# drtconway/zotmer

Measured on AMD Instinct MI355X. Metric: Gk-mers/sec kmerize k=25 on synthetic 150bp FASTQ; achieved HBM GB/s fraction, higher is better.
Workload: dtype u64

## Files before the change

include/zotk.h:

```cpp
#ifndef ZOTK_H
#define ZOTK_H

#include <stdint.h>

#ifdef __cplusplus
extern "C" {
#endif

#define ZK_OK 0
#define ZK_EINVAL (-1)
#define ZK_ENOMEM (-2)
#define ZK_EHIP (-3)
#define ZK_ENOSPC (-4)
#define ZK_EOVERFLOW (-5)
#define ZK_EINTERNAL (-6)
#define ZK_ERANGE (-7)

typedef struct zk_ctx zk_ctx;

zk_ctx* zk_create(int device, uint64_t workspace_bytes);
void zk_destroy(zk_ctx* ctx);
const char* zk_last_error(zk_ctx* ctx);
int zk_set_stream(zk_ctx* ctx, void* hip_stream);
void* zk_get_stream(zk_ctx* ctx);
// ... 9 lines not shown
int zk_host_alloc(zk_ctx* ctx, uint64_t bytes, void** ptr);
int zk_host_free(zk_ctx* ctx, void* ptr);
int zk_upload_async(zk_ctx* ctx, void* d_dst, const void* src, uint64_t bytes);

#define ZK_TUNE_SORT_VARIANT 1
#define ZK_TUNE_PAIRS_VARIANT 2
#define ZK_TUNE_SHORT_SORT 3
#define ZK_TUNE_XCD_GROUP 5
#define ZK_TUNE_SIDE_DIV 4
#define ZK_TUNE_EARLY_COLLAPSE 7
#define ZK_TUNE_PACKED_PAIRS 8
#define ZK_TUNE_WIDE_TILES 9
#define ZK_TUNE_STREAM_PASS 10
#define ZK_TUNE_STREAM_RANGES 11
#define ZK_TUNE_TAG_WORDS 12
#define ZK_TUNE_DEDUPE_VARIANT 13
#define ZK_TUNE_DEDUPE_LIMIT 14
#define ZK_TUNE_DEDUPE_BITS 15
#define ZK_TUNE_COMM_CHUNK 6
#define ZK_TUNE_TAG_PASS 17
#define ZK_TUNE_KWAY 18
#define ZK_TUNE_TILE_SORT 19
#define ZK_TUNE_STRAND_BLOCKS 20
#define ZK_TUNE_COMM_SELF_LOOP 16
int zk_tune(zk_ctx* ctx, int what, int value);

#define ZK_PROF_HIST_STREAM 1
#define ZK_PROF_HIST_ARRAY 2
#define ZK_PROF_PASS_STREAM 3
#define ZK_PROF_PASS_KEYS 4
#define ZK_PROF_PASS_PAIRS 5
#define ZK_PROF_RLE 6
#define ZK_PROF_UNION 7
#define ZK_PROF_SELECT 8
#define ZK_PROF_MIRROR 9
#define ZK_PROF_INTERSECT 10
#define ZK_PROF_COUNT_HIST 11
#define ZK_PROF_PASS_PACKED 12
#define ZK_PROF_SAMPLE 13
#define ZK_PROF_TILE_SORT 14
#define ZK_PROF_CAPTURE_HITS 15
#define ZK_PROF_PROJECT_SUM 16
#define ZK_PROF_SPECTRUM 17
#define ZK_PROF_STRAND_KEYS 18
#define ZK_PROF_STRAND_PAIRS 19
#define ZK_PROF_FORMAT_PAIRS 20
// ... 259 lines not shown
```

zotmer_amd/csrc/context.hip:

```cpp
#include <stdarg.h>
#include <string.h>

#include "internal.hpp"
#include <vector>

namespace zk {

int fail(zk_ctx* c, int code, const char* fmt, ...) {
    char buf[512];
    va_list ap;
    va_start(ap, fmt);
    vsnprintf(buf, sizeof buf, fmt, ap);
    va_end(ap);
    if (c) c->last_error = buf;
    return code;
}

void arena_reset(zk_ctx* c) { c->arena_off = 0; }

int arena_alloc(zk_ctx* c, uint64_t bytes, void** p) {
    const uint64_t need = (bytes + 255) & ~255ull;
    if (c->arena_off + need > c->arena_size) {
        if (c->arena_off != 0)
            return fail(c, ZK_ENOMEM, "workspace too small: %llu bytes in use, %llu more needed, %llu reserved (call zk_reserve)",
// ... 285 lines not shown
    if (what == ZK_TUNE_SHORT_SORT) { c->short_sort = value; return ZK_OK; }
    if (what == ZK_TUNE_SIDE_DIV) { c->side_div = value; return ZK_OK; }
    if (what == ZK_TUNE_WIDE_TILES) { c->wide_tiles = value ? 1 : 0; return ZK_OK; }
    if (what == ZK_TUNE_PACKED_PAIRS) { c->packed_pairs = value ? 1 : 0; return ZK_OK; }
    if (what == ZK_TUNE_EARLY_COLLAPSE) { c->early_collapse = value < 0 ? 0 : (value > 3 ? 3 : value); return ZK_OK; }
    if (what == ZK_TUNE_COMM_SELF_LOOP) { c->comm_self_loop = value ? 1 : 0; return ZK_OK; }
    if (what == ZK_TUNE_COMM_CHUNK) { c->comm_chunk_bytes = value > 0 ? (uint64_t)value : 0; return ZK_OK; }
    if (what == ZK_TUNE_STREAM_PASS) {
#ifdef ZK_PHASES
        c->stream_pass = value < 0 ? 0 : value;
#else
        if (value < 0 || value > 3) return fail(c, ZK_EINVAL, "stream pass variant %d (0, 1, 2 or 3)", value);
        c->stream_pass = value;
#endif
        return ZK_OK;
    }
    if (what == ZK_TUNE_TAG_WORDS) { c->tag_words = value < 0 ? 0 : (value > 2 ? 2 : value); return ZK_OK; }
    if (what == ZK_TUNE_DEDUPE_VARIANT) { c->dedupe_variant = value < 0 ? -1 : (value & 3); return ZK_OK; }
    if (what == ZK_TUNE_KWAY) { c->kway = value < 0 ? 0 : (value > 2 ? 2 : value); return ZK_OK; }
    if (what == ZK_TUNE_TILE_SORT) { c->tile_sort = value ? 1 : 0; return ZK_OK; }
    if (what == ZK_TUNE_TAG_PASS) { c->tag_pass = value ? 1 : 0; return ZK_OK; }
    if (what == ZK_TUNE_DEDUPE_BITS) { c->dedupe_bits = value < 0 ? 0 : value; return ZK_OK; }
    if (what == ZK_TUNE_STRAND_BLOCKS) { c->strand_blocks = value < 0 ? 0 : (value > 3 ? 1 : value); return ZK_OK; }
    if (what == ZK_TUNE_DEDUPE_LIMIT) { c->dedupe_limit = value < 1 ? 1 : (value > 65536 ? 65536 : value); return ZK_OK; }
    if (what == ZK_TUNE_STREAM_RANGES) { c->stream_ranges = value < 0 ? 0 : (value > 4096 ? 4096 : value); return ZK_OK; }
    if (what == ZK_TUNE_XCD_GROUP) {
        if (value < 0 || value > 32 || (value & (value - 1))) return fail(c, ZK_EINVAL, "xcd group must be 0 or a power of two <= 32");
        c->xcd_group = value;
        return ZK_OK;
    }
    return fail(c, ZK_EINVAL, "unknown tuning knob %d", what);
}

int zk_debug_buffer(zk_ctx* c, void* d_buf) {
    if (!c) return ZK_EINVAL;
    enter(c);
    c->dbg = (u64*)d_buf;
    return ZK_OK;
}

int zk_profile(zk_ctx* c, int enable) {
    if (!c) return ZK_EINVAL;
    enter(c);
    ZK_HIP(c, hipStreamSynchronize(c->stream));
    for (auto& r : c->prof) { (void)hipEventDestroy(r.a); (void)hipEventDestroy(r.b); }
    c->prof.clear();
// ... 91 lines not shown
```

zotmer_amd/csrc/dedupe2.hip:

```cpp
#include "dedupe.hpp"
#include <type_traits>

namespace zk {

template <int BLOCK_, int BATCH_, int ITEMS_>
struct Dedupe2Smem {
    static constexpr int BLOCK = BLOCK_, BATCH = BATCH_, ITEMS = ITEMS_, TILE = BLOCK * ITEMS, NW = BLOCK / 64, ALL = 11264, SPT = ALL / BLOCK,
                         NB = 1024, SIDE = 64 + 64 * BATCH;
    static_assert(ALL % BLOCK == 0 && ALL % 8 == 0 && ITEMS % BATCH == 0 && ITEMS % 4 == 0, "whole rounds, whole quads, whole batches");
    alignas(16) u32 keys[ALL];
    alignas(16) u32 cnt[ALL / 2];
    union {
        u32 side[NW][SIDE];
        struct { u32 bc[NB]; u32 bbase[NB + 1]; } g;
    };
    u32 ticket;
    u32 nout;
};

template <int ITEMS>
struct Dedupe2Next {
    u32 chunk;
    u64 lo;
    u32 len;
// ... 283 lines not shown
        st.len = nhi - nlo < (u64)a.limit ? (u32)(nhi - nlo) : ~0u;
    }
    if (st.len - 1u < ~0u - 1u) dedupe2_load<BLOCK, ITEMS, TAGIN>(a, st.lo, 0, st.len, tmask, st.tag);
    __syncthreads();
    u32 ph[8] = {0, 0, 0, 0, 0, 0, 0, 0};
    u32 tlast = a.dbg ? (u32)__builtin_amdgcn_s_memtime() : 0u;
    (void)tlast;
    u32 nblk = 0;
    while (st.chunk < a.chunks) {
        dedupe2_block<BLOCK, BATCH, ITEMS, TAGIN, UNSORTED>(a, sm, st, ph, tlast);
        __syncthreads();
        DD_PHASE(6);
        nblk++;
    }
    if (a.dbg && threadIdx.x == 0 && blockIdx.x < 256) {
        for (int k = 0; k < 8; k++) a.dbg[(u64)blockIdx.x * 16 + k] = ph[k];
        a.dbg[(u64)blockIdx.x * 16 + 8] = nblk;
    }
}

int launch_dedupe2(zk_ctx* c, const DedupeArgs& a, bool tagin, int variant, bool unsorted) {
    const u32 want = 2u * (u32)c->num_cus;
    const u32 grid = a.chunks < want ? a.chunks : want;
#define ZK_DD2(N, T, U) hipLaunchKernelGGL((dedupe2_kernel<512, N, 8, T, U>), dim3(grid), dim3(512), 0, c->stream, a)
#define ZK_DD2B(T, U) switch (variant & 3) { case 1: ZK_DD2(1, T, U); break; case 2: ZK_DD2(2, T, U); break; default: ZK_DD2(4, T, U); break; }
    if (unsorted) {
        if (tagin) ZK_DD2B(true, true) else ZK_DD2B(false, true)
    } else {
        if (tagin) ZK_DD2B(true, false) else ZK_DD2B(false, false)
    }
#undef ZK_DD2B
#undef ZK_DD2
    ZK_HIP(c, hipGetLastError());
    return ZK_OK;
}

}
```

zotmer_amd/csrc/internal.hpp:

```cpp
#pragma once
#include <hip/hip_runtime.h>
#include <stddef.h>
#include <stdint.h>
#include <stdio.h>
#include <string>
#include <vector>

#include "../../include/zotk.h"
#include "common.hpp"

struct zk_strand_counters { u32 n_declined, fail; };
struct zk_scalars {
    u64 rle_side;
    u64 total;
    u64 acgt[4];
    u64 n_keys;
    u64 rec_info[3];
    u64 sample_n;
    u64 dedupe_flags, dedupe_n_retry, dedupe_counter, dedupe_n_big, dedupe_n_bad;
    u64 dedupe_n_in;
    u64 dedupe_n_out;
    zk_strand_counters strand;
    u64 hist_big_n;
    u64 capture_kept;
// ... 44 lines not shown
              ZK_SPAN(dedupe_flags, dedupe_n_bad) == 5 * sizeof(u64), "dedupe_pass clears and reads its five words as one range");

struct zk_ctx {
    int device = 0;
    hipStream_t stream = nullptr;
    bool own_stream = false;
    int num_cus = 256;
    int sort_variant = 3;
    int short_sort = 0;
    int packed_pairs = 1;
    int wide_tiles = 1;
    int early_collapse = 1;
    int side_div = 8;
    int pairs_variant = 7;
    int stream_pass = 1;
    int tag_words = 2;
    int dedupe_variant = 0;
    int dedupe_limit = 65536;
    int tag_pass = 0;
    int kway = 1;
    int tile_sort = 1;
    int dedupe_bits = 0;
    int strand_blocks = 1;
    int stream_ranges = 0;

    char* arena = nullptr;
    uint64_t arena_size = 0;
    uint64_t arena_off = 0;

    char* aux = nullptr;
    uint64_t aux_size = 0;

    u64* status = nullptr;
    uint64_t status_words = 0;
    unsigned short* part16 = nullptr;
    uint64_t part16_words = 0;
    u32 epoch = 0;
    u32* d_ticket = nullptr;
    u32* d_xticket = nullptr;
    int num_xcd = 1;
    int xcd_group = 0;
    u32 ticket_base = 0;

    u32* d_err = nullptr;
    zk_scalars* d_scalars = nullptr;
    zk_scalars* h_scalars = nullptr;
// ... 73 lines not shown
        p.shift[i] = s;
        s += p.bits[i];
    }
    return p;
}
int sort_keys(zk_ctx* c, u64* keys, u64* alt, uint64_t n, int key_bits, u64** result);
int sort_pairs(zk_ctx* c, u64* keys, u64* alt, u32* vals, u32* valt, uint64_t n, int key_bits, u64** rk, u32** rv);
int sort_keys_upper(zk_ctx* c, u64* keys, u64* alt, uint64_t n, int key_bits, int lo_bit, u64** result, int prof_tag = ZK_PROF_PASS_PACKED);
int sort_pairs_upper(zk_ctx* c, u64* keys, u64* alt, u32* vals, u32* valt, uint64_t n, int key_bits, int lo_bit, u64** rk, u32** rv);
int sort_pairs_mirrored(zk_ctx* c, const u64* src_k, const u32* src_v, u64* keys, u64* alt, u32* vals, u32* valt, uint64_t n, int K,
                        u64** rk, u32** rv, int lo_bit = 0);
int sort_pairs_rbits(zk_ctx* c);
struct StreamSample { int shift; uint64_t value; double max_ratio; uint64_t seen = 0, distinct = 0; bool want_distinct = false; };
struct StreamTags { bool written = false; u64* cuts = nullptr; uint32_t blocks = 0; };
struct StreamSrc { const u8* stream; uint64_t n_bytes; int K; int mode; int lo_bit; int hi_bit = 0; StreamSample* sample = nullptr;
                   StreamTags* tags = nullptr; };
int sort_stream(zk_ctx* c, const StreamSrc& src, u64* buf_a, u64* buf_b, uint64_t cap, uint64_t* n_keys,
                uint64_t acgt[4], u64** result);
int sort_rbits(zk_ctx* c);
PassPlan sort_plan_upper(zk_ctx* c, int key_bits, int lo_bit);
int sort_first_bits(zk_ctx* c, int key_bits, int lo_bit);
constexpr int MIRROR_RBITS = 9, MIRROR_RADIX = 1 << MIRROR_RBITS;
struct MirrorHist { int passes; int shift[4]; int bits[4]; u64* raw; };
int sort_keys_upper_counted(zk_ctx* c, u64* keys, u64* alt, uint64_t n, int key_bits, int lo_bit, u64* counted, u64** result);
struct DedupeResult {
    uint64_t n_out = 0;
    uint32_t flags = 0;
    uint32_t n_big = 0;
    u64 *cuts = nullptr, *nwords = nullptr, *incl = nullptr, *big = nullptr, *work = nullptr;
    u32* sub = nullptr;
    uint32_t chunks = 0;
    int pack = 0;
    int tag_bits = 0;
    bool unsorted = false;
};
int dedupe_pass(zk_ctx* c, const u64* keys, uint64_t n, int key_bits, int b, int pack, u64* work, uint64_t cap, DedupeResult* r,
                uint64_t* n_in = nullptr, uint64_t max_chunks = 0, const u32* tags = nullptr, const u64* tag_cuts = nullptr,
                bool unsorted = false);
int expand_tags(zk_ctx* c, const u32* tags, const u64* cuts, uint32_t blocks, int tag_bits, u64* keys_out, uint64_t first_block = 0, uint64_t n_blocks = 0);
int dedupe_finish(zk_ctx* c, const DedupeResult& r, u64* out_k, u32* out_c, u64* out_m = nullptr, int K = 0, int gbases = 0,
                  u64** mirror_hist = nullptr, int* mirror_group_bits = nullptr, bool packed_out = false);
int dedupe_sort_blocks(zk_ctx* c, DedupeResult& r);
int strand_blocks(zk_ctx* c, const DedupeResult& r, u64* keys_buf, uint64_t buf_words, int K, u64* out_k, u32* out_c, uint64_t cap,
                  uint64_t* n_out);
int collapse_pass(zk_ctx* c, const u64* keys, uint64_t n, int shift, int bits, int pack, u64* out, uint64_t cap, uint64_t* n_out,
                  uint64_t max_tiles = 0);
struct StreamRows { u32* rows = nullptr; u64* offs = nullptr; u32 ranges = 0, radix = 0; u32* gcodes = nullptr; u16* gvalid = nullptr;
// ... 61 lines not shown
```

zotmer_amd/csrc/radix_sort.hip:

```cpp
#include <stdlib.h>
#include "internal.hpp"
#include "encode_tile.hpp"

namespace zk {

constexpr int MAX_RADIX = 1024;

enum { SRC_ARRAY = 0, SRC_STREAM = 1 };

template <int BLOCK_, int ITEMS_, int RBITS_, int ROUNDS_ = 1, int WPE_ = 1, int SEG_ = 32, bool PIPE_ = false>
struct Cfg {
    static constexpr int BLOCK = BLOCK_, ITEMS = ITEMS_, RBITS = RBITS_, ROUNDS = ROUNDS_, WPE = WPE_, SEG = SEG_;
    static constexpr bool PIPE = PIPE_;
    static_assert(SEG == 0 || (BLOCK * ITEMS < 32768 && (SEG & (SEG - 1)) == 0), "16-bit tile counts");
    static constexpr int TILE = BLOCK * ITEMS, RADIX = 1 << RBITS, NW = BLOCK / 64;
    static constexpr int EXCH = TILE / ROUNDS, IPR = ITEMS / ROUNDS;
    static_assert(ITEMS % ROUNDS == 0, "ROUNDS");
    static constexpr int DPT = (RADIX + BLOCK - 1) / BLOCK;
    static_assert(ITEMS % 2 == 0 && 2 * ITEMS < 256, "ITEMS");
    static_assert(64 * ITEMS < 65536, "per-wave ranks are 16-bit");
    static_assert(RADIX <= MAX_RADIX && RBITS * MAX_PASSES >= 64, "RBITS");
};

struct SortArgs {
// ... 1207 lines not shown
        if (SRC == SRC_STREAM && src.n_bytes) {
            h.rec_info = c->d_scalars->rec_info;
            ZK_HIP(c, hipMemsetAsync(h.rec_info, 0, 3 * sizeof(u64), c->stream));
            hipLaunchKernelGGL(first_newline_kernel, dim3(1), dim3(256), 0, c->stream, src.stream, (u64)src.n_bytes, h.rec_info);
        }
        if (acgt) ZK_HIP(c, hipMemsetAsync(acgt, 0, sizeof(u64) * 4, c->stream));
        u32 grid = grid_cap(c, h.tiles, 8);
        if (grid == 0) grid = 1;
        prof_begin(c, SRC == SRC_STREAM ? ZK_PROF_HIST_STREAM : ZK_PROF_HIST_ARRAY, SRC == SRC_STREAM ? src.n_bytes : 8 * src.n);
        if constexpr (SRC == SRC_STREAM && C::ITEMS == 16 && C::BLOCK <= 512) {
            if (src.mode != ZK_KEYS_BOTH) hipLaunchKernelGGL((hist_kernel<C, SRC, true>), dim3(grid), dim3(C::BLOCK), 0, c->stream, h);
            else hipLaunchKernelGGL((hist_kernel<C, SRC, false>), dim3(grid), dim3(C::BLOCK), 0, c->stream, h);
        } else {
            hipLaunchKernelGGL((hist_kernel<C, SRC, false>), dim3(grid), dim3(C::BLOCK), 0, c->stream, h);
        }
        prof_end(c);
        ZK_HIP(c, hipGetLastError());
        hipLaunchKernelGGL(hist_scan_kernel, dim3(1), dim3(256), 0, c->stream, ghist, plan.passes, (int)C::RADIX, d_n);
        ZK_HIP(c, hipGetLastError());
        return ZK_OK;
    }

    static int sort_keys(zk_ctx* c, u64* keys, u64* alt, uint64_t n, int key_bits, u64** result, int lo_bit = 0, int prof_tag = 0,
                         u64* counted = nullptr) {
        PassPlan plan = make_plan(key_bits - lo_bit, C::RBITS, lo_bit);
        u64* ghist = counted;
        if (!counted) ZK_TRY(arena_alloc(c, sizeof(u64) * MAX_PASSES * C::RADIX, (void**)&ghist));
        SortArgs a = {};
        a.kin = keys; a.n = n;
        a.prof_tag = prof_tag;
        if (counted) {
            hipLaunchKernelGGL(hist_scan_kernel, dim3(1), dim3(256), 0, c->stream, ghist, plan.passes, (int)C::RADIX, &c->d_scalars->n_keys);
            ZK_HIP(c, hipGetLastError());
        } else {
            ZK_TRY(launch_hist<SRC_ARRAY>(c, a, plan, ghist, nullptr, &c->d_scalars->n_keys));
        }
        u64* in = keys; u64* out = alt;
        for (int p = 0; p < plan.passes; p++) {
            a.kin = in; a.kout = out; a.shift = plan.shift[p]; a.bits = plan.bits[p];
            a.ghist = ghist + p * C::RADIX;
            ZK_TRY(launch_keys_pass(c, a));
            u64* t = in; in = out; out = t;
        }
        *result = in;
        return ZK_OK;
    }

    static int sort_pairs(zk_ctx* c, u64* keys, u64* alt, u32* vals, u32* valt, uint64_t n, int key_bits, u64** rk, u32** rv,
                          const u64* src_k = nullptr, const u32* src_v = nullptr, int mirror_K = 0, int lo_bit = 0, bool unordered = false) {
        PassPlan plan = make_plan(key_bits - lo_bit, C::RBITS, lo_bit);
        u64* ghist;
        ZK_TRY(arena_alloc(c, sizeof(u64) * MAX_PASSES * C::RADIX, (void**)&ghist));
        SortArgs a = {};
        a.kin = mirror_K ? src_k : keys; a.n = n; a.mirror_K = mirror_K;
        ZK_TRY(launch_hist<SRC_ARRAY>(c, a, plan, ghist, nullptr, &c->d_scalars->n_keys));
        const u64* in = mirror_K ? src_k : keys; const u32* vi = mirror_K ? src_v : vals;
        u64* out = mirror_K ? keys : alt; u32* vo = mirror_K ? vals : valt;
        for (int p = 0; p < plan.passes; p++) {
            a.kin = in; a.kout = out; a.vin = vi; a.vout = vo; a.shift = plan.shift[p]; a.bits = plan.bits[p];
            a.ghist = ghist + p * C::RADIX;
            a.mirror_K = (p == 0) ? mirror_K : 0;
            if constexpr (PIPE_PAIRS) {
                a.straddle = nullptr;
// ... 208 lines not shown

int sort_pairs(zk_ctx* c, u64* keys, u64* alt, u32* vals, u32* valt, uint64_t n, int key_bits, u64** rk, u32** rv) {
    *rk = keys; *rv = vals;
    if (n == 0) return ZK_OK;
    const int top = c->tile_sort ? tile_sort_top_bits(n, key_bits, sort_pairs_rbits(c)) : 0;
    if (top) {
        u64* k1 = nullptr; u32* v1 = nullptr;
        bool declined = false;
        ZK_TRY(sort_pairs_upper(c, keys, alt, vals, valt, n, key_bits, key_bits - top, &k1, &v1));
        ZK_TRY(tile_sort(c, k1, v1, n, key_bits, top, &declined));
        *rk = k1; *rv = v1;
        if (!declined) return ZK_OK;
        return sort_pairs_lsd(c, k1, k1 == keys ? alt : keys, v1, v1 == vals ? valt : vals, n, key_bits, rk, rv);
    }
    return sort_pairs_lsd(c, keys, alt, vals, valt, n, key_bits, rk, rv);
}

int sort_keys_upper(zk_ctx* c, u64* keys, u64* alt, uint64_t n, int key_bits, int lo_bit, u64** result, int prof_tag) {
    *result = keys;
    if (n == 0 || lo_bit >= key_bits) return ZK_OK;
    ZK_SORT_DISPATCH(c, sort_keys(c, keys, alt, n, key_bits, result, lo_bit, prof_tag));
}

int sort_keys_upper_counted(zk_ctx* c, u64* keys, u64* alt, uint64_t n, int key_bits, int lo_bit, u64* counted, u64** result) {
    *result = keys;
    if (n == 0 || lo_bit >= key_bits) return ZK_OK;
    return Sorter<V3>::sort_keys(c, keys, alt, n, key_bits, result, lo_bit, ZK_PROF_PASS_PACKED, counted);
}

int sort_pairs_upper(zk_ctx* c, u64* keys, u64* alt, u32* vals, u32* valt, uint64_t n, int key_bits, int lo_bit, u64** rk, u32** rv) {
    *rk = keys; *rv = vals;
    if (n == 0) return ZK_OK;
    ZK_PAIRS_DISPATCH(c, sort_pairs(c, keys, alt, vals, valt, n, key_bits, rk, rv, nullptr, nullptr, 0, lo_bit));
}

int sort_pairs_mirrored(zk_ctx* c, const u64* src_k, const u32* src_v, u64* keys, u64* alt, u32* vals, u32* valt, uint64_t n, int K,
                        u64** rk, u32** rv, int lo_bit) {
    *rk = keys; *rv = vals;
    if (n == 0) return ZK_OK;
    ZK_PAIRS_DISPATCH(c, sort_pairs(c, keys, alt, vals, valt, n, 2 * K, rk, rv, src_k, src_v, K, lo_bit, true));
}

int sort_rbits(zk_ctx* c) { ZK_SORT_DISPATCH(c, rbits()); }
int sort_pairs_rbits(zk_ctx* c) { ZK_PAIRS_DISPATCH(c, rbits()); }

PassPlan sort_plan_upper(zk_ctx* c, int key_bits, int lo_bit) { return make_plan(key_bits - lo_bit, sort_rbits(c), lo_bit); }

int sort_first_bits(zk_ctx* c, int key_bits, int lo_bit) {
    if (lo_bit >= key_bits) return 0;
    return make_plan(key_bits - lo_bit, sort_rbits(c), lo_bit).bits[0];
// ... 14 lines not shown
```

zotmer_amd/csrc/strand_blocks.hip:

```cpp
#include "tile_group.hpp"

namespace zk {

constexpr int SB_ITEMS = 16, SB_GROUPS = 2048;
constexpr u32 SB_GROUP_MAX = 128;
typedef TileSortSmem<SB_ITEMS, SB_GROUPS, false> StrandSmem;
constexpr int SB_BLOCK_BITS = 18;

__global__ __launch_bounds__(256) void strand_mirror_kernel(const u64* __restrict__ in, const u64* __restrict__ cuts, const u64* __restrict__ incl,
                                                            const u64* __restrict__ nwords, u32 chunks, int pack, int K, u64* __restrict__ out_m,
                                                            MirrorHist mh) {
    __shared__ u32 bins[4 * 512];
    const bool hist = mh.passes > 0;
    if (hist) {
        for (int q = threadIdx.x; q < 4 * 512; q += blockDim.x) bins[q] = 0;
        __syncthreads();
    }
    const u64 maxc = (1ull << pack) - 1;
    for (u32 v = blockIdx.x; v < chunks; v += gridDim.x) {
        const u64 cnt = nwords[v];
        const u64 dst0 = incl[v] - cnt;
        const u64* src = in + cuts[v];
        for (u64 i0 = threadIdx.x; i0 < cnt; i0 += 4ull * blockDim.x) {
            u64 w4[4];
#pragma unroll
            for (int q = 0; q < 4; q++) {
                const u64 i = i0 + (u64)q * blockDim.x;
                w4[q] = i < cnt ? src[i] : 0;
            }
// ... 22 lines not shown
    const u32 g = blockIdx.x * blockDim.x + threadIdx.x;
    if (g > (1u << SB_BLOCK_BITS)) return;
    u64 lo = 0, hi = n;
    if (g == (1u << SB_BLOCK_BITS)) lo = n;
    while (lo < hi) {
        const u64 mid = (lo + hi) >> 1;
        if ((m[mid] >> shift) < (u64)g) lo = mid + 1; else hi = mid;
    }
    start[g] = lo;
}

struct StrandArgs {
    const u64* cw;
    const u64* cuts; const u64* nwords; const u64* incl;
    const u64* m;
    const u64* mstart;
    u64* ok; u32* oc;
    int pack;
    int pshift;
    u32* n_declined;
    u32* declined;
};

__device__ __forceinline__ bool strand_crowded(const StrandSmem& sm, int tid) {
    static_assert(SB_GROUPS == 4 * TS_BLOCK, "four groups a thread");
    u32 big = 0;
#pragma unroll
    for (int q = 0; q < 4; q++) big |= sm.start[4 * tid + q + 1] - sm.start[4 * tid + q] > SB_GROUP_MAX ? 1u : 0u;
    return __syncthreads_or((int)big) != 0;
}

__device__ __forceinline__ void strand_write(const StrandSmem& sm, const TileMap& tm, u32 m, u64* ok, u32* oc, int pack, int tid) {
    const u64 maxc = (1ull << pack) - 1;
    constexpr int E = 2;
    for (u32 i0 = (u32)tid; i0 < m; i0 += E * TS_BLOCK) {
        u32 i[E], place[E];
        u64 mine[E];
#pragma unroll
        for (int e = 0; e < E; e++) i[e] = i0 + e * TS_BLOCK;
        tile_rank<E, false>(sm, tm, i, m, mine, place);
#pragma unroll
        for (int e = 0; e < E; e++) {
            if (i[e] >= m) break;
            ok[place[e]] = mine[e] >> pack;
            oc[place[e]] = (u32)(mine[e] & maxc);
        }
    }
}

__global__ __launch_bounds__(TS_BLOCK, 2 * TS_BLOCK / 256) void strand_block_union_kernel(StrandArgs a) {
    using S = StrandSmem;
    constexpr u32 CAP = S::CAP;
    static_assert(sizeof(S) <= 80 * 1024, "two workgroups per CU");
    __shared__ S sm;
    const u32 b = blockIdx.x;
    const u64 nc = a.nwords[b], m0 = a.mstart[b], nm = a.mstart[b + 1] - m0;
    const u64 n = nc + nm;
    if (n == 0) return;
    if (n > CAP) {
        if (threadIdx.x == 0) a.declined[atomicAdd(a.n_declined, 1u)] = b;
        return;
    }
    int tid = threadIdx.x;
    asm volatile("" : "+v"(tid));
    const u32 m = (u32)n;
    const TileMap tm = tile_group<SB_ITEMS, SB_GROUPS, false>(sm, a.cw, nullptr, a.cuts[b], m, a.pshift, tid, a.m, m0, (u32)nc);
    if (strand_crowded(sm, tid)) {
        if (tid == 0) a.declined[atomicAdd(a.n_declined, 1u)] = b;
        return;
    }
    const u64 out0 = a.incl[b] - nc + m0;
    strand_write(sm, tm, m, a.ok + out0, a.oc + out0, a.pack, tid);
}

constexpr int SB_SPLIT = 256;
struct StrandBigSmem {
    StrandSmem t;
    u64 sp[SB_SPLIT];
    u32 cnt[SB_SPLIT + 2];
    u32 tile[SB_SPLIT + 2];
    u32 ntiles, gcount, fail;
};

__global__ __launch_bounds__(TS_BLOCK) void strand_big_block_kernel(StrandArgs a, u32 n_list, u64* __restrict__ scratch, u32* __restrict__ fail) {
    using S = StrandBigSmem;
    constexpr u32 CAP = StrandSmem::CAP, R = SB_SPLIT + 1;
    __shared__ S sm;
    u64* gat = scratch + (u64)blockIdx.x * CAP;
    const int lane = threadIdx.x & 63;
    for (u32 li = blockIdx.x; li < n_list; li += gridDim.x) {
        int tid = threadIdx.x;
        asm volatile("" : "+v"(tid));
        const u32 b = a.declined[li];
        const u64 nc = a.nwords[b], m0 = a.mstart[b], nm = a.mstart[b + 1] - m0, n = nc + nm;
        const u64* C = a.cw + a.cuts[b];
// ... 122 lines not shown
    if (uc == 0) return ZK_OK;
    if (!(K & 1) || r.n_big || r.chunks != (1u << SB_BLOCK_BITS)) return fail(c, ZK_EINTERNAL, "strand_blocks: K %d, %u big counts, %u blocks", K, r.n_big, r.chunks);
    const uint64_t a8w = ((8 * uc + 255) & ~255ull) / 8;
    if (2 * a8w > buf_words) return fail(c, ZK_EINTERNAL, "strand_blocks: %llu words do not fit twice in %llu", (unsigned long long)uc, (unsigned long long)buf_words);
    if (2 * uc > cap) return fail(c, ZK_ENOSPC, "output holds %llu entries, the table has %llu", (unsigned long long)cap, (unsigned long long)(2 * uc));
    const int pk = r.pack, key_bits = 2 * K + pk, lo_bit = key_bits - SB_BLOCK_BITS;
    u64* mw = keys_buf;
    u64* malt = keys_buf + a8w;
    MirrorHist mh = {};
    if (c->sort_variant == 3) {
        const PassPlan plan = sort_plan_upper(c, key_bits, lo_bit);
        if (plan.passes <= 4) {
            ZK_TRY(arena_alloc(c, sizeof(u64) * MAX_PASSES * 512, (void**)&mh.raw));
            ZK_HIP(c, hipMemsetAsync(mh.raw, 0, sizeof(u64) * MAX_PASSES * 512, c->stream));
            mh.passes = plan.passes;
            for (int p = 0; p < plan.passes; p++) { mh.shift[p] = plan.shift[p]; mh.bits[p] = plan.bits[p]; }
        }
    }
    prof_begin(c, ZK_PROF_SELECT, 16 * uc);
    hipLaunchKernelGGL(strand_mirror_kernel, dim3((u32)c->num_cus * 8), dim3(256), 0, c->stream, r.work, r.cuts, r.incl, r.nwords, r.chunks, pk, K, mw, mh);
    prof_end(c);
    ZK_HIP(c, hipGetLastError());
    u64* sk = nullptr;
    if (mh.passes) ZK_TRY(sort_keys_upper_counted(c, mw, malt, uc, key_bits, lo_bit, mh.raw, &sk));
    else ZK_TRY(sort_keys_upper(c, mw, malt, uc, key_bits, lo_bit, &sk));
    u64* mstart;
    u32* declined;
    ZK_TRY(arena_alloc(c, sizeof(u64) * ((1ull << SB_BLOCK_BITS) + 1), (void**)&mstart));
    ZK_TRY(arena_alloc(c, sizeof(u32) * r.chunks, (void**)&declined));
    StrandArgs a = {};
    a.cw = r.work; a.cuts = r.cuts; a.nwords = r.nwords; a.incl = r.incl; a.m = sk; a.mstart = mstart;
    a.ok = out_k; a.oc = out_c; a.pack = pk; a.pshift = lo_bit;
    a.n_declined = &c->d_scalars->strand.n_declined;
    a.declined = declined;
    u32* fail = &c->d_scalars->strand.fail;
    prof_begin(c, ZK_PROF_UNION, 8 * 2 * uc + 12 * 2 * uc);
    hipLaunchKernelGGL(strand_starts_kernel, dim3(((1u << SB_BLOCK_BITS) + 256) / 256), dim3(256), 0, c->stream, sk, (u64)uc, lo_bit, mstart);
    ZK_HIP(c, hipMemsetAsync(&c->d_scalars->strand, 0, sizeof(zk_strand_counters), c->stream));
    hipLaunchKernelGGL(strand_block_union_kernel, dim3(r.chunks), dim3(TS_BLOCK), 0, c->stream, a);
    prof_end(c);
    ZK_HIP(c, hipGetLastError());
    ZK_TRY(fetch(c, &c->h_scalars->strand));
    ZK_TRY(check_device_error(c));
    const uint32_t n_declined = c->h_scalars->strand.n_declined;
    bool other_way = n_declined && c->strand_blocks == 3;
    if (n_declined && !other_way) {
        const uint32_t grid = n_declined < 2u * (uint32_t)c->num_cus ? n_declined : 2u * (uint32_t)c->num_cus;
        u64* scratch;
        ZK_TRY(arena_alloc(c, sizeof(u64) * StrandSmem::CAP * grid, (void**)&scratch));
        prof_begin(c, ZK_PROF_UNION, 0);
        hipLaunchKernelGGL(strand_big_block_kernel, dim3(grid), dim3(TS_BLOCK), 0, c->stream, a, n_declined, scratch, fail);
        prof_end(c);
        ZK_HIP(c, hipGetLastError());
        ZK_TRY(fetch(c, &c->h_scalars->strand));
        ZK_TRY(check_device_error(c));
        other_way = c->h_scalars->strand.fail != 0;
    }
    if (!other_way) {
        *n_out = 2 * uc;
        return ZK_OK;
    }
    DedupeResult rs = r;
// ... 11 lines not shown
```

zotmer_amd/csrc/tile_group.hpp:

```cpp
#pragma once
#include "internal.hpp"

namespace zk {

constexpr int TS_BLOCK = 512;
constexpr u32 TS_SLACK = 1024;

template <int ITEMS, int GROUPS, bool PAIRS>
struct TileSortSmem {
    static constexpr int CAP = TS_BLOCK * ITEMS;
    alignas(16) u64 keys[CAP];
    u32 vals[PAIRS ? CAP : 1];
    u16 idx[PAIRS ? CAP : 1];
    alignas(16) u32 start[GROUPS + 8];
    u32 wsum[TS_BLOCK / 64];
};
struct TileMap {
    u64 kmin; int sh; u32 scale;
    __device__ __forceinline__ u32 group(u64 key) const {
        const u32 d = (u32)((key - kmin) >> sh);
        return scale ? __umulhi(d, scale) : d;
    }
};

template <int ITEMS, int G, bool PAIRS, class S>
__device__ __forceinline__ TileMap tile_group(S& sm, const u64* kin, const u32* vin, u64 lo, u32 m, int pshift, int tid,
                                              const u64* kin2 = nullptr, u64 lo2 = 0, u32 m1 = ~0u, bool ranged = false, u64 vlo = 0,
                                              u64 vhi = 0) {
    constexpr int NW = TS_BLOCK / 64, QPT = G / TS_BLOCK / 4;
    static_assert(QPT == 1 || QPT == 2, "four or eight groups a thread in the scan");
    static_assert((S::CAP <= 8192 || (!PAIRS && S::CAP <= 16384)) && G <= 4096, "group | place << 12 in a word; u16 places of pairs");
    const int lane = tid & 63, wave = __builtin_amdgcn_readfirstlane(tid >> 6);
    const u64* kp = kin + lo;
    u64 k[ITEMS];
    u32 v[PAIRS ? ITEMS : 1];
#pragma unroll
    for (int j = 0; j < ITEMS; j++) {
        const u32 i = (u32)j * TS_BLOCK + tid;
        k[j] = i < m ? (i < m1 ? kp[i] : kin2[lo2 + (i - m1)]) : ~0ull;
        if constexpr (PAIRS) v[j] = i < m ? vin[lo + i] : 0u;
    }
    u64 first, last;
    if (ranged) { first = vlo; last = vhi; pshift = 0; }
    else { first = m1 ? kp[0] : kin2[lo2]; last = m - 1 < m1 ? kp[m - 1] : kin2[lo2 + (m - 1 - m1)]; }
    TileMap tm;
    tm.kmin = (first >> pshift) << pshift;
    const u64 rm1 = (((last >> pshift) - (first >> pshift)) << pshift) | ((1ull << pshift) - 1ull);
    tm.sh = rm1 >> 32 ? 32 - __builtin_clzll(rm1) : 0;
    const u32 rs = (u32)(rm1 >> tm.sh);
    tm.scale = rs < (u32)G ? 0u : (u32)(((u64)G << 32) / ((u64)rs + 1ull));
    {
        uint4* z = reinterpret_cast<uint4*>(sm.start);
#pragma unroll
        for (int q = 0; q < QPT; q++) z[QPT * tid + q] = make_uint4(0, 0, 0, 0);
    }
    __syncthreads();
    u32 gp[ITEMS];
#pragma unroll
    for (int j = 0; j < ITEMS; j++) {
        const u32 i = (u32)j * TS_BLOCK + tid;
        const u32 g = i < m ? tm.group(k[j]) : 0u;
        gp[j] = g;
        if (i < m) gp[j] |= atomicAdd(&sm.start[g], 1u) << 12;
    }
    __syncthreads();
    {
        uint4* z = reinterpret_cast<uint4*>(sm.start);
        uint4 cq[QPT];
        u32 sum = 0;
#pragma unroll
        for (int q = 0; q < QPT; q++) { cq[q] = z[QPT * tid + q]; sum += cq[q].x + cq[q].y + cq[q].z + cq[q].w; }
        const u32 inc = wave_incl_scan_u32(sum);
        if (lane == 63) sm.wsum[wave] = inc;
        __syncthreads();
        u32 run = inc - sum;
#pragma unroll
        for (int w = 0; w < NW; w++) run += w < wave ? sm.wsum[w] : 0u;
#pragma unroll
        for (int q = 0; q < QPT; q++) {
            uint4 sq;
            sq.x = run; run += cq[q].x; sq.y = run; run += cq[q].y; sq.z = run; run += cq[q].z; sq.w = run; run += cq[q].w;
            z[QPT * tid + q] = sq;
        }
        if (tid == 0) sm.start[G] = m;
    }
    __syncthreads();
#pragma unroll
    for (int j = 0; j < ITEMS; j++) {
        const u32 i = (u32)j * TS_BLOCK + tid;
        if (i < m) {
            const u32 p = sm.start[gp[j] & (G - 1)] + (gp[j] >> 12);
            sm.keys[p] = k[j];
            if constexpr (PAIRS) { sm.vals[p] = v[j]; sm.idx[p] = (u16)i; }
        }
    }
    __syncthreads();
    return tm;
}

template <int E, bool PAIRS, class S>
__device__ __forceinline__ void tile_rank(const S& sm, const TileMap& tm, const u32 (&i)[E], u32 m, u64 (&mine)[E], u32 (&place)[E]) {
    constexpr u32 CAP = S::CAP;
    auto before = [&](u64 ko, u32 q, u64 km, u32 at) -> bool {
        if (ko != km) return ko < km;
        if constexpr (PAIRS) return q != at && sm.idx[q] < sm.idx[at];
        else return q < at;
    };
    u32 g0[E], g1[E];
#pragma unroll
    for (int e = 0; e < E; e++) mine[e] = sm.keys[i[e] < m ? i[e] : 0u];
#pragma unroll
    for (int e = 0; e < E; e++) {
// ... 33 lines not shown
```

zotmer_amd/native.py:

```python
import ctypes as C
import os

import numpy as np

_HERE = os.path.dirname(os.path.abspath(__file__))
LIB_PATH = os.environ.get("ZOTK_LIB") or os.path.join(_HERE, "libzotk.so")

ZK_OK, ZK_EINVAL, ZK_ENOMEM, ZK_EHIP, ZK_ENOSPC, ZK_EOVERFLOW, ZK_EINTERNAL, ZK_ERANGE = 0, -1, -2, -3, -4, -5, -6, -7
KMERIZE_CANONICAL, KMERIZE_BOTH, KMERIZE_SUBSAMPLE, KMERIZE_CANONICAL_ONLY = 0, 1, 2, 4
STRAND_ORPHANS = 1
PROBE_TILE, PROBE_MAX_WINDOWS = 4096, 1024
TALLY_TILE = 2048
CONTIG_TILE = 4096
VARS_TILE = 4096
LINKS_TILE = 1024
NO_LINK = 0xFFFFFFFF
PILEUP_DIAGS, PILEUP_TILE = 256, 4096
PATH_TILE, PATH_CHUNK = 4096, 256
DEFAULT_TAG_WORDS = 2

_ERRNAMES = {-1: "ZK_EINVAL", -2: "ZK_ENOMEM", -3: "ZK_EHIP", -4: "ZK_ENOSPC", -5: "ZK_EOVERFLOW",
             -6: "ZK_EINTERNAL", -7: "ZK_ERANGE"}


class ZotkError(RuntimeError):
    def __init__(self, code, msg):
        super().__init__("%s: %s" % (_ERRNAMES.get(code, code), msg))
        self.code = code


class Spectrum(C.Structure):
    _fields_ = [("n_shared", C.c_uint64), ("s_min", C.c_uint64), ("x_shared", C.c_uint64), ("y_shared", C.c_uint64),
                ("s_xy_lo", C.c_uint64), ("s_xy_hi", C.c_uint64), ("s_sqrt", C.c_double), ("s_js", C.c_double)]


class StrandStats(C.Structure):
    _fields_ = [("n_pairs", C.c_uint64), ("n_orphans", C.c_uint64), ("n_palindromes", C.c_uint64)]


class ContigStats(C.Structure):
    _fields_ = [("n_records", C.c_uint64), ("n_windows", C.c_uint64), ("n_keys", C.c_uint64), ("n_bins", C.c_uint64)]

# ... 351 lines not shown
        return cut.value

    def device_to_file(self, arr, fileno, offset, threads=None):
        self._check(self.lib.zk_device_to_file(self.h, arr.ptr, arr.nbytes, int(fileno), int(offset), threads or self.IO_THREADS))

    def file_to_device(self, fileno, offset, nbytes, dtype=np.uint8, threads=None):
        dt = np.dtype(dtype)
        out = self.empty(nbytes // dt.itemsize, dt)
        self._check(self.lib.zk_file_to_device(self.h, int(fileno), int(offset), int(nbytes), out.ptr, threads or self.IO_THREADS))
        return out

    def upload_stream(self, data):
        a = np.frombuffer(data, dtype=np.uint8) if isinstance(data, (bytes, bytearray, memoryview)) else np.asarray(data, np.uint8)
        return self.upload(a)

    PROF_TAGS = {"hist_stream": 1, "hist_array": 2, "pass_stream": 3, "pass_keys": 4, "pass_pairs": 5, "rle": 6,
                 "union_sum": 7, "select": 8, "mirror": 9, "intersect": 10, "count_hist": 11, "pass_packed": 12, "sample": 13, "tile_sort": 14,
                 "capture_hits": 15, "project_sum": 16, "spectrum": 17, "strand_keys": 18, "strand_pairs": 19, "format_pairs": 20,
                 "probe_scan": 21, "bait_tally": 22, "vars_scan": 23, "links": 24, "links_rc": 25, "contig_render": 26,
                 "pileup": 27, "pileup_cut": 28, "pulldown_tally": 29, "capture_kmers": 30, "path_scan": 31}

    TUNE_IDS = dict(sort_variant=1, pairs_variant=2, short_sort=3, side_div=4, xcd_group=5, comm_chunk=6, early_collapse=7,
                    packed_pairs=8, wide_tiles=9, stream_pass=10, stream_ranges=11, tag_words=12, dedupe_variant=13, dedupe_limit=14,
                    dedupe_bits=15, comm_self_loop=16, tag_pass=17, kway=18, tile_sort=19, strand_blocks=20)

    def tune(self, **knobs):
        for name in knobs:
            if name not in self.TUNE_IDS:
                raise TypeError("tune() got an unexpected keyword argument %r" % name)
        for name, value in knobs.items():
            if value is not None:
                self._check(self.lib.zk_tune(self.h, self.TUNE_IDS[name], int(value)))

    def profile(self, enable=True):
        self._check(self.lib.zk_profile(self.h, int(enable)))

    def profile_read(self):
        out = {}
        for name, tag in self.PROF_TAGS.items():
            n, b, ms = C.c_uint64(0), C.c_uint64(0), C.c_double(0)
            self._check(self.lib.zk_profile_read(self.h, tag, C.byref(n), C.byref(ms), C.byref(b)))
            if n.value:
                out[name] = dict(launches=n.value, ms=ms.value, bytes=b.value)
        return out

    def pack_reads(self, bases, offs):
        n_reads = offs.n - 1
# ... 575 lines not shown
```

Measured before the change: 165.2.

## Add strand_wide knob: unordered upper sort straddle, 1024-thread strand and dedupe kernels

Adds a strand_wide tuning knob with three bits. Bit 1, on by default, makes the strand path's upper-bits key sort run unordered and build straddle bitmaps for its first two passes. Bits 2 and 4, off by default, switch the unsorted dedupe and strand block-union kernels to 1024-thread workgroups, and tile_group is generalised over block size to support them. The default path aims to drop ordering work in the strand sort, at the cost of extra bitmap allocation and launches.

```diff
diff --git a/include/zotk.h b/include/zotk.h
--- a/include/zotk.h
+++ b/include/zotk.h
@@ -55,6 +55,7 @@
 #define ZK_TUNE_KWAY 18
 #define ZK_TUNE_TILE_SORT 19
 #define ZK_TUNE_STRAND_BLOCKS 20
+#define ZK_TUNE_STRAND_WIDE 21
 #define ZK_TUNE_COMM_SELF_LOOP 16
 int zk_tune(zk_ctx* ctx, int what, int value);
 
diff --git a/zotmer_amd/csrc/context.hip b/zotmer_amd/csrc/context.hip
--- a/zotmer_amd/csrc/context.hip
+++ b/zotmer_amd/csrc/context.hip
@@ -331,6 +331,7 @@
     if (what == ZK_TUNE_TAG_PASS) { c->tag_pass = value ? 1 : 0; return ZK_OK; }
     if (what == ZK_TUNE_DEDUPE_BITS) { c->dedupe_bits = value < 0 ? 0 : value; return ZK_OK; }
     if (what == ZK_TUNE_STRAND_BLOCKS) { c->strand_blocks = value < 0 ? 0 : (value > 3 ? 1 : value); return ZK_OK; }
+    if (what == ZK_TUNE_STRAND_WIDE) { c->strand_wide = value < 0 ? 0 : (value & 7); return ZK_OK; }
     if (what == ZK_TUNE_DEDUPE_LIMIT) { c->dedupe_limit = value < 1 ? 1 : (value > 65536 ? 65536 : value); return ZK_OK; }
     if (what == ZK_TUNE_STREAM_RANGES) { c->stream_ranges = value < 0 ? 0 : (value > 4096 ? 4096 : value); return ZK_OK; }
     if (what == ZK_TUNE_XCD_GROUP) {
diff --git a/zotmer_amd/csrc/dedupe2.hip b/zotmer_amd/csrc/dedupe2.hip
--- a/zotmer_amd/csrc/dedupe2.hip
+++ b/zotmer_amd/csrc/dedupe2.hip
@@ -329,6 +329,12 @@
 int launch_dedupe2(zk_ctx* c, const DedupeArgs& a, bool tagin, int variant, bool unsorted) {
     const u32 want = 2u * (u32)c->num_cus;
     const u32 grid = a.chunks < want ? a.chunks : want;
+    if (unsorted && (c->strand_wide & 2)) {
+        if (tagin) hipLaunchKernelGGL((dedupe2_kernel<1024, 2, 8, true, true>), dim3(grid), dim3(1024), 0, c->stream, a);
+        else hipLaunchKernelGGL((dedupe2_kernel<1024, 2, 8, false, true>), dim3(grid), dim3(1024), 0, c->stream, a);
+        ZK_HIP(c, hipGetLastError());
+        return ZK_OK;
+    }
 #define ZK_DD2(N, T, U) hipLaunchKernelGGL((dedupe2_kernel<512, N, 8, T, U>), dim3(grid), dim3(512), 0, c->stream, a)
 #define ZK_DD2B(T, U) switch (variant & 3) { case 1: ZK_DD2(1, T, U); break; case 2: ZK_DD2(2, T, U); break; default: ZK_DD2(4, T, U); break; }
     if (unsorted) {
diff --git a/zotmer_amd/csrc/internal.hpp b/zotmer_amd/csrc/internal.hpp
--- a/zotmer_amd/csrc/internal.hpp
+++ b/zotmer_amd/csrc/internal.hpp
@@ -90,6 +90,7 @@
     int tile_sort = 1;
     int dedupe_bits = 0;
     int strand_blocks = 1;
+    int strand_wide = 1;
     int stream_ranges = 0;
 
     char* arena = nullptr;
@@ -209,7 +210,8 @@
 int sort_first_bits(zk_ctx* c, int key_bits, int lo_bit);
 constexpr int MIRROR_RBITS = 9, MIRROR_RADIX = 1 << MIRROR_RBITS;
 struct MirrorHist { int passes; int shift[4]; int bits[4]; u64* raw; };
-int sort_keys_upper_counted(zk_ctx* c, u64* keys, u64* alt, uint64_t n, int key_bits, int lo_bit, u64* counted, u64** result);
+int sort_keys_upper_counted(zk_ctx* c, u64* keys, u64* alt, uint64_t n, int key_bits, int lo_bit, u64* counted, u64** result,
+                            bool unordered = false);
 struct DedupeResult {
     uint64_t n_out = 0;
     uint32_t flags = 0;
diff --git a/zotmer_amd/csrc/radix_sort.hip b/zotmer_amd/csrc/radix_sort.hip
--- a/zotmer_amd/csrc/radix_sort.hip
+++ b/zotmer_amd/csrc/radix_sort.hip
@@ -1253,7 +1253,7 @@
     }
 
     static int sort_keys(zk_ctx* c, u64* keys, u64* alt, uint64_t n, int key_bits, u64** result, int lo_bit = 0, int prof_tag = 0,
-                         u64* counted = nullptr) {
+                         u64* counted = nullptr, bool unordered = false) {
         PassPlan plan = make_plan(key_bits - lo_bit, C::RBITS, lo_bit);
         u64* ghist = counted;
         if (!counted) ZK_TRY(arena_alloc(c, sizeof(u64) * MAX_PASSES * C::RADIX, (void**)&ghist));
@@ -1270,6 +1270,9 @@
         for (int p = 0; p < plan.passes; p++) {
             a.kin = in; a.kout = out; a.shift = plan.shift[p]; a.bits = plan.bits[p];
             a.ghist = ghist + p * C::RADIX;
+            a.straddle = nullptr;
+            if (C::PIPE && unordered && p <= 1)
+                ZK_TRY(straddle_bitmap(c, n, keys_pass_tile(c), p == 1 ? ghist : nullptr, 1u << plan.bits[0], (u32)C::RADIX, &a.straddle));
             ZK_TRY(launch_keys_pass(c, a));
             u64* t = in; in = out; out = t;
         }
@@ -1524,10 +1527,10 @@
     ZK_SORT_DISPATCH(c, sort_keys(c, keys, alt, n, key_bits, result, lo_bit, prof_tag));
 }
 
-int sort_keys_upper_counted(zk_ctx* c, u64* keys, u64* alt, uint64_t n, int key_bits, int lo_bit, u64* counted, u64** result) {
+int sort_keys_upper_counted(zk_ctx* c, u64* keys, u64* alt, uint64_t n, int key_bits, int lo_bit, u64* counted, u64** result, bool unordered) {
     *result = keys;
     if (n == 0 || lo_bit >= key_bits) return ZK_OK;
-    return Sorter<V3>::sort_keys(c, keys, alt, n, key_bits, result, lo_bit, ZK_PROF_PASS_PACKED, counted);
+    return Sorter<V3>::sort_keys(c, keys, alt, n, key_bits, result, lo_bit, ZK_PROF_PASS_PACKED, counted, unordered);
 }
 
 int sort_pairs_upper(zk_ctx* c, u64* keys, u64* alt, u32* vals, u32* valt, uint64_t n, int key_bits, int lo_bit, u64** rk, u32** rv) {
diff --git a/zotmer_amd/csrc/strand_blocks.hip b/zotmer_amd/csrc/strand_blocks.hip
--- a/zotmer_amd/csrc/strand_blocks.hip
+++ b/zotmer_amd/csrc/strand_blocks.hip
@@ -5,6 +5,9 @@
 constexpr int SB_ITEMS = 16, SB_GROUPS = 2048;
 constexpr u32 SB_GROUP_MAX = 128;
 typedef TileSortSmem<SB_ITEMS, SB_GROUPS, false> StrandSmem;
+constexpr int SB_WIDE_BLOCK = 1024;
+typedef TileSortSmem<SB_ITEMS * TS_BLOCK / SB_WIDE_BLOCK, SB_GROUPS, false, SB_WIDE_BLOCK> StrandWideSmem;
+static_assert(StrandWideSmem::CAP == StrandSmem::CAP, "one tile size: a block declined by either is strand_big_block_kernel's");
 constexpr int SB_BLOCK_BITS = 18;
 
 __global__ __launch_bounds__(256) void strand_mirror_kernel(const u64* __restrict__ in, const u64* __restrict__ cuts, const u64* __restrict__ incl,
@@ -73,22 +76,25 @@
     u32* declined;
 };
 
-__device__ __forceinline__ bool strand_crowded(const StrandSmem& sm, int tid) {
-    static_assert(SB_GROUPS == 4 * TS_BLOCK, "four groups a thread");
+template <int BLOCK = TS_BLOCK, class S>
+__device__ __forceinline__ bool strand_crowded(const S& sm, int tid) {
+    constexpr int GPT = SB_GROUPS / BLOCK;
+    static_assert(SB_GROUPS == GPT * BLOCK, "whole groups a thread");
     u32 big = 0;
 #pragma unroll
-    for (int q = 0; q < 4; q++) big |= sm.start[4 * tid + q + 1] - sm.start[4 * tid + q] > SB_GROUP_MAX ? 1u : 0u;
+    for (int q = 0; q < GPT; q++) big |= sm.start[GPT * tid + q + 1] - sm.start[GPT * tid + q] > SB_GROUP_MAX ? 1u : 0u;
     return __syncthreads_or((int)big) != 0;
 }
 
-__device__ __forceinline__ void strand_write(const StrandSmem& sm, const TileMap& tm, u32 m, u64* ok, u32* oc, int pack, int tid) {
+template <int BLOCK = TS_BLOCK, class S>
+__device__ __forceinline__ void strand_write(const S& sm, const TileMap& tm, u32 m, u64* ok, u32* oc, int pack, int tid) {
     const u64 maxc = (1ull << pack) - 1;
     constexpr int E = 2;
-    for (u32 i0 = (u32)tid; i0 < m; i0 += E * TS_BLOCK) {
+    for (u32 i0 = (u32)tid; i0 < m; i0 += E * BLOCK) {
         u32 i[E], place[E];
         u64 mine[E];
 #pragma unroll
-        for (int e = 0; e < E; e++) i[e] = i0 + e * TS_BLOCK;
+        for (int e = 0; e < E; e++) i[e] = i0 + e * BLOCK;
         tile_rank<E, false>(sm, tm, i, m, mine, place);
 #pragma unroll
         for (int e = 0; e < E; e++) {
@@ -99,9 +105,11 @@
     }
 }
 
-__global__ __launch_bounds__(TS_BLOCK, 2 * TS_BLOCK / 256) void strand_block_union_kernel(StrandArgs a) {
-    using S = StrandSmem;
+template <int BLOCK>
+__global__ __launch_bounds__(BLOCK, 2 * BLOCK / 256) void strand_block_union_kernel(StrandArgs a) {
+    using S = std::conditional_t<BLOCK == TS_BLOCK, StrandSmem, StrandWideSmem>;
     constexpr u32 CAP = S::CAP;
+    constexpr int ITEMS = (int)CAP / BLOCK;
     static_assert(sizeof(S) <= 80 * 1024, "two workgroups per CU");
     __shared__ S sm;
     const u32 b = blockIdx.x;
@@ -115,13 +123,13 @@
     int tid = threadIdx.x;
     asm volatile("" : "+v"(tid));
     const u32 m = (u32)n;
-    const TileMap tm = tile_group<SB_ITEMS, SB_GROUPS, false>(sm, a.cw, nullptr, a.cuts[b], m, a.pshift, tid, a.m, m0, (u32)nc);
-    if (strand_crowded(sm, tid)) {
+    const TileMap tm = tile_group<ITEMS, SB_GROUPS, false, BLOCK>(sm, a.cw, nullptr, a.cuts[b], m, a.pshift, tid, a.m, m0, (u32)nc);
+    if (strand_crowded<BLOCK>(sm, tid)) {
         if (tid == 0) a.declined[atomicAdd(a.n_declined, 1u)] = b;
         return;
     }
     const u64 out0 = a.incl[b] - nc + m0;
-    strand_write(sm, tm, m, a.ok + out0, a.oc + out0, a.pack, tid);
+    strand_write<BLOCK>(sm, tm, m, a.ok + out0, a.oc + out0, a.pack, tid);
 }
 
 constexpr int SB_SPLIT = 256;
@@ -290,7 +298,7 @@
     prof_end(c);
     ZK_HIP(c, hipGetLastError());
     u64* sk = nullptr;
-    if (mh.passes) ZK_TRY(sort_keys_upper_counted(c, mw, malt, uc, key_bits, lo_bit, mh.raw, &sk));
+    if (mh.passes) ZK_TRY(sort_keys_upper_counted(c, mw, malt, uc, key_bits, lo_bit, mh.raw, &sk, (c->strand_wide & 1) != 0));
     else ZK_TRY(sort_keys_upper(c, mw, malt, uc, key_bits, lo_bit, &sk));
     u64* mstart;
     u32* declined;
@@ -305,7 +313,8 @@
     prof_begin(c, ZK_PROF_UNION, 8 * 2 * uc + 12 * 2 * uc);
     hipLaunchKernelGGL(strand_starts_kernel, dim3(((1u << SB_BLOCK_BITS) + 256) / 256), dim3(256), 0, c->stream, sk, (u64)uc, lo_bit, mstart);
     ZK_HIP(c, hipMemsetAsync(&c->d_scalars->strand, 0, sizeof(zk_strand_counters), c->stream));
-    hipLaunchKernelGGL(strand_block_union_kernel, dim3(r.chunks), dim3(TS_BLOCK), 0, c->stream, a);
+    if (c->strand_wide & 4) hipLaunchKernelGGL(strand_block_union_kernel<SB_WIDE_BLOCK>, dim3(r.chunks), dim3(SB_WIDE_BLOCK), 0, c->stream, a);
+    else hipLaunchKernelGGL(strand_block_union_kernel<TS_BLOCK>, dim3(r.chunks), dim3(TS_BLOCK), 0, c->stream, a);
     prof_end(c);
     ZK_HIP(c, hipGetLastError());
     ZK_TRY(fetch(c, &c->h_scalars->strand));
diff --git a/zotmer_amd/csrc/tile_group.hpp b/zotmer_amd/csrc/tile_group.hpp
--- a/zotmer_amd/csrc/tile_group.hpp
+++ b/zotmer_amd/csrc/tile_group.hpp
@@ -1,19 +1,20 @@
 #pragma once
 #include "internal.hpp"
+#include <type_traits>
 
 namespace zk {
 
 constexpr int TS_BLOCK = 512;
 constexpr u32 TS_SLACK = 1024;
 
-template <int ITEMS, int GROUPS, bool PAIRS>
+template <int ITEMS, int GROUPS, bool PAIRS, int BLOCK = TS_BLOCK>
 struct TileSortSmem {
-    static constexpr int CAP = TS_BLOCK * ITEMS;
+    static constexpr int CAP = BLOCK * ITEMS;
     alignas(16) u64 keys[CAP];
     u32 vals[PAIRS ? CAP : 1];
     u16 idx[PAIRS ? CAP : 1];
     alignas(16) u32 start[GROUPS + 8];
-    u32 wsum[TS_BLOCK / 64];
+    u32 wsum[BLOCK / 64];
 };
 struct TileMap {
     u64 kmin; int sh; u32 scale;
@@ -23,12 +24,15 @@
     }
 };
 
-template <int ITEMS, int G, bool PAIRS, class S>
+template <int ITEMS, int G, bool PAIRS, int BLOCK = TS_BLOCK, class S>
 __device__ __forceinline__ TileMap tile_group(S& sm, const u64* kin, const u32* vin, u64 lo, u32 m, int pshift, int tid,
                                               const u64* kin2 = nullptr, u64 lo2 = 0, u32 m1 = ~0u, bool ranged = false, u64 vlo = 0,
                                               u64 vhi = 0) {
-    constexpr int NW = TS_BLOCK / 64, QPT = G / TS_BLOCK / 4;
-    static_assert(QPT == 1 || QPT == 2, "four or eight groups a thread in the scan");
+    constexpr int NW = BLOCK / 64, GPT = G / BLOCK;
+    static_assert(G % BLOCK == 0 && (GPT == 2 || GPT == 4 || GPT == 8), "two, four or eight groups a thread in the scan");
+    static_assert(S::CAP == BLOCK * ITEMS, "the tile of this workgroup");
+    using GV = std::conditional_t<GPT == 2, uint2, uint4>;
+    constexpr int VPT = GPT == 2 ? 1 : GPT / 4, VW = GPT == 2 ? 2 : 4;
     static_assert((S::CAP <= 8192 || (!PAIRS && S::CAP <= 16384)) && G <= 4096, "group | place << 12 in a word; u16 places of pairs");
     const int lane = tid & 63, wave = __builtin_amdgcn_readfirstlane(tid >> 6);
     const u64* kp = kin + lo;
@@ -36,7 +40,7 @@
     u32 v[PAIRS ? ITEMS : 1];
 #pragma unroll
     for (int j = 0; j < ITEMS; j++) {
-        const u32 i = (u32)j * TS_BLOCK + tid;
+        const u32 i = (u32)j * BLOCK + tid;
         k[j] = i < m ? (i < m1 ? kp[i] : kin2[lo2 + (i - m1)]) : ~0ull;
         if constexpr (PAIRS) v[j] = i < m ? vin[lo + i] : 0u;
     }
@@ -50,26 +54,33 @@
     const u32 rs = (u32)(rm1 >> tm.sh);
     tm.scale = rs < (u32)G ? 0u : (u32)(((u64)G << 32) / ((u64)rs + 1ull));
     {
-        uint4* z = reinterpret_cast<uint4*>(sm.start);
+        GV* z = reinterpret_cast<GV*>(sm.start);
+        GV zero;
+        zero.x = 0; zero.y = 0;
+        if constexpr (VW == 4) { zero.z = 0; zero.w = 0; }
 #pragma unroll
-        for (int q = 0; q < QPT; q++) z[QPT * tid + q] = make_uint4(0, 0, 0, 0);
+        for (int q = 0; q < VPT; q++) z[VPT * tid + q] = zero;
     }
     __syncthreads();
     u32 gp[ITEMS];
 #pragma unroll
     for (int j = 0; j < ITEMS; j++) {
-        const u32 i = (u32)j * TS_BLOCK + tid;
+        const u32 i = (u32)j * BLOCK + tid;
         const u32 g = i < m ? tm.group(k[j]) : 0u;
         gp[j] = g;
         if (i < m) gp[j] |= atomicAdd(&sm.start[g], 1u) << 12;
     }
     __syncthreads();
     {
-        uint4* z = reinterpret_cast<uint4*>(sm.start);
-        uint4 cq[QPT];
+        GV* z = reinterpret_cast<GV*>(sm.start);
+        GV cq[VPT];
         u32 sum = 0;
 #pragma unroll
-        for (int q = 0; q < QPT; q++) { cq[q] = z[QPT * tid + q]; sum += cq[q].x + cq[q].y + cq[q].z + cq[q].w; }
+        for (int q = 0; q < VPT; q++) {
+            cq[q] = z[VPT * tid + q];
+            sum += cq[q].x + cq[q].y;
+            if constexpr (VW == 4) sum += cq[q].z + cq[q].w;
+        }
         const u32 inc = wave_incl_scan_u32(sum);
         if (lane == 63) sm.wsum[wave] = inc;
         __syncthreads();
@@ -77,17 +88,18 @@
 #pragma unroll
         for (int w = 0; w < NW; w++) run += w < wave ? sm.wsum[w] : 0u;
 #pragma unroll
-        for (int q = 0; q < QPT; q++) {
-            uint4 sq;
-            sq.x = run; run += cq[q].x; sq.y = run; run += cq[q].y; sq.z = run; run += cq[q].z; sq.w = run; run += cq[q].w;
-            z[QPT * tid + q] = sq;
+        for (int q = 0; q < VPT; q++) {
+            GV sq;
+            sq.x = run; run += cq[q].x; sq.y = run; run += cq[q].y;
+            if constexpr (VW == 4) { sq.z = run; run += cq[q].z; sq.w = run; run += cq[q].w; }
+            z[VPT * tid + q] = sq;
         }
         if (tid == 0) sm.start[G] = m;
     }
     __syncthreads();
 #pragma unroll
     for (int j = 0; j < ITEMS; j++) {
-        const u32 i = (u32)j * TS_BLOCK + tid;
+        const u32 i = (u32)j * BLOCK + tid;
         if (i < m) {
             const u32 p = sm.start[gp[j] & (G - 1)] + (gp[j] >> 12);
             sm.keys[p] = k[j];
diff --git a/zotmer_amd/native.py b/zotmer_amd/native.py
--- a/zotmer_amd/native.py
+++ b/zotmer_amd/native.py
@@ -18,6 +18,7 @@
 PILEUP_DIAGS, PILEUP_TILE = 256, 4096
 PATH_TILE, PATH_CHUNK = 4096, 256
 DEFAULT_TAG_WORDS = 2
+DEFAULT_STRAND_WIDE = 1
 
 _ERRNAMES = {-1: "ZK_EINVAL", -2: "ZK_ENOMEM", -3: "ZK_EHIP", -4: "ZK_ENOSPC", -5: "ZK_EOVERFLOW",
              -6: "ZK_EINTERNAL", -7: "ZK_ERANGE"}
@@ -415,7 +416,7 @@
 
     TUNE_IDS = dict(sort_variant=1, pairs_variant=2, short_sort=3, side_div=4, xcd_group=5, comm_chunk=6, early_collapse=7,
                     packed_pairs=8, wide_tiles=9, stream_pass=10, stream_ranges=11, tag_words=12, dedupe_variant=13, dedupe_limit=14,
-                    dedupe_bits=15, comm_self_loop=16, tag_pass=17, kway=18, tile_sort=19, strand_blocks=20)
+                    dedupe_bits=15, comm_self_loop=16, tag_pass=17, kway=18, tile_sort=19, strand_blocks=20, strand_wide=21)
 
     def tune(self, **knobs):
         for name in knobs:
```

Result: no change. 166.3 (median of 6 runs) (+0.7%).
